# biodatageeks/datafusion-bio-functions

Hardware: AMD Instinct MI355X
Metric: overlap-pairs/sec + probe-rows/sec, IntervalJoinExec 100Mx1M (higher is better)
Workload: dtype int32; 1 GPU; join_100Mx1M_24contigs; probe_rows_per_gpu=100000000, build_rows_per_gpu=1000000, contigs=24, pairs_per_gpu=37210484, parallelism=partition-per-gpu x1, gather=False, build_overlap=True

## Files before the change

datafusion-bio-functions_amd/csrc/ivx_regions_probe.hip:

```cpp
#include "ivx_regions.hpp"
#include "ivx_agg.hpp"
#include "ivx_select.hpp"
#include "ivx_where.hpp"

namespace {


#ifndef IVX_RP_B
#define IVX_RP_B 8
#endif
#ifndef IVX_RP_RING
#define IVX_RP_RING 512
#endif
constexpr int RP_B = IVX_RP_B;
constexpr u32 RP_HALO = IVX_RP_HALO;
constexpr u32 RP_CCAP = 8192 + RP_HALO + 2;
constexpr u32 RP_RING = IVX_RP_RING;
constexpr u32 RP_NSLOT = 4;
constexpr u32 RP_NPG = 64;
constexpr u32 RP_STASH = 48;
constexpr u32 FD_SLOT_SHIFT = 13;
#ifndef IVX_FD_HEAD
#define IVX_FD_HEAD 3
#endif
constexpr int FD_HEAD = IVX_FD_HEAD;
static_assert(RP_ECAP <= (1u << FD_SLOT_SHIFT), "a slice slot must fit a stash entry's j field");
constexpr u32 RP_GRID = 256;
#ifndef IVX_RP_VGRID
#define IVX_RP_VGRID 512
#endif
constexpr u32 RP_VGRID = IVX_RP_VGRID;

struct Slice {
    const JoinIndexView *ix;
    const unsigned short *s_off; const u64 *s_ent; const u32 *s_row;
    u32 sh0, nlev, k, lb, slo, shi, e0, ncell0; bool inlds, upper, lev0;
    i32 origin; u32 span;
    i32 rbase;
    bool fast; u32 off, cmax, ncm1;
};

template <class F>
__device__ __forceinline__ void probe_row(const Slice &S, i32 qs, i32 qe, F &&f)
{
    const JoinIndexView &ix = *S.ix;
    const i64 hi64 = (i64)qe - (i64)S.origin;
    if (hi64 < 0) return;
    if (S.lev0) {
        const u32 ncell = S.ncell0;
        const i64 lo64 = (i64)qs - ((i64)1 << S.sh0) + 1 - (i64)S.origin;
        const i64 bl = lo64 <= 0 ? 0 : (lo64 >> S.sh0);
        if (bl < (i64)ncell) {
            const u32 blo = (u32)bl;
            const i64 bh = hi64 >> S.sh0;
            const u32 bhi = bh >= (i64)ncell ? ncell - 1u : (u32)bh;
            if (blo <= bhi) {
                if (S.inlds && blo >= S.slo && bhi < S.shi) {
                    const u32 a = S.s_off[blo - S.slo], b = S.s_off[bhi + 1 - S.slo];
                    for (u32 j = a; j < b; j++) {
                        const u64 x = S.s_ent[j];
                        if ((i32)(u32)x <= qe && (i32)(u32)(x >> 32) >= qs) f(j, true, (i32)(u32)x, (i32)(u32)(x >> 32));
                    }
                } else {
                    const u32 a = ix.binstart[S.lb + blo], b = ix.binstart[S.lb + bhi + 1];
                    for (u32 j = a; j < b; j++) {
                        const ivx_ent x = ix.ent[j];
                        if (x.s <= qe && x.e >= qs) f(x.row, false, x.s, x.e);
                    }
                }
            }
        }
    }
    if (S.upper) {
        for (u32 l = 1; l < S.nlev; l++) {
            if (ix.hdr[HDR_LEVCNT + l] == 0) continue;
            const u32 sh = S.sh0 + IVX_LSTEP * l;
            u32 blo = 0, bhi = 0;
            if (sh < 32) {
                const u32 ncell = (S.span >> sh) + 1u;
                const i64 lo64 = (i64)qs - ((i64)1 << sh) + 1 - (i64)S.origin;
                const i64 bl = lo64 <= 0 ? 0 : (lo64 >> sh);
                const i64 bh = hi64 >> sh;
                if (bl >= (i64)ncell) continue;
                blo = (u32)bl;
                bhi = bh >= (i64)ncell ? ncell - 1u : (u32)bh;
                if (blo > bhi) continue;
            }
            const u32 base = ix.lbase[(u64)l * ix.nkeys + S.k];
            const u32 a = ix.binstart[base + blo], b = ix.binstart[base + bhi + 1];
            for (u32 j = a; j < b; j++) {
                const ivx_ent x = ix.ent[j];
                if (x.s <= qe && x.e >= qs) f(x.row, false, x.s, x.e);
            }
        }
    }
}

template <class F>
__device__ __forceinline__ void probe_row_rel(const Slice &S, u32 rel, u32 len, bool ok, i32 qs, i32 qe, F &&f)
{
    if (S.fast && ok) {
        const u32 t = ((rel + 1u) >> S.sh0) + S.off;
        const u32 bl = t ? t - 1u : 0u;
        u32 bh = ((rel + len) >> S.sh0) + S.off;
        bh = bh < S.cmax ? bh : S.cmax;
        if (bh < S.ncm1) {
            if (bl <= bh) {
                const u32 a = S.s_off[bl], b = S.s_off[bh + 1u];
                for (u32 j = a; j < b; j++) {
                    const u64 x = S.s_ent[j];
                    if ((i32)(u32)x <= qe && (i32)(u32)(x >> 32) >= qs) f(j, true, (i32)(u32)x, (i32)(u32)(x >> 32));
                }
            }
            return;
        }
    }
    probe_row(S, qs, qe, f);
}


struct ProbeLds {
    unsigned short *s_off; u64 *s_ent; u32 *s_row;
    u64 (*s_q)[RP_RING];
    u32 *s_wpos;
    u32 (*s_wcnt)[RP_W];
    unsigned long long *s_base;
    u32 *s_arrive, *s_ready;
};

__device__ __forceinline__ void slice_init(const JoinIndexView &ix, Slice &S, const ProbeLds &L)
{
    S.ix = &ix; S.s_off = L.s_off; S.s_ent = L.s_ent; S.s_row = L.s_row;
    S.sh0 = ix.hdr[HDR_SH0]; S.nlev = ix.hdr[HDR_NLEV];
    S.upper = false;
    for (u32 l = 1; l < S.nlev; l++) S.upper |= ix.hdr[HDR_LEVCNT + l] != 0;
    S.lev0 = ix.hdr[HDR_LEVCNT] != 0;
}

__device__ __forceinline__ void slice_load(const JoinIndexView &ix, Slice &S, const ProbeLds &L, u32 r, bool reload)
{
    const u32 tid = threadIdx.x;
    __syncthreads();
    const ivx_regdesc d = ix.rdesc[r];
    S.k = d.k; S.origin = d.origin; S.span = d.span; S.lb = d.lb;
    S.ncell0 = (S.span >> S.sh0) + 1u;
    S.slo = d.slo; S.shi = d.shi; S.e0 = d.e0; S.rbase = d.rbase;
    const u32 ne = d.ne;
    const u32 nc = S.shi - S.slo + 1u;
    S.inlds = ne <= RP_ECAP && nc <= RP_CCAP;
    S.fast = S.inlds && S.lev0 && !S.upper;
    S.off = (u32)(((i64)S.rbase - (i64)S.origin) >> S.sh0) - S.slo;
    S.cmax = S.ncell0 - 1u - S.slo; S.ncm1 = S.shi - S.slo;
    if (S.inlds && reload) {
        for (u32 c0 = 0; c0 < nc; c0 += RP_T * 4) {
            u32 v[4];
#pragma unroll
            for (int u = 0; u < 4; u++) { const u32 c = c0 + u * RP_T + tid; v[u] = c < nc ? ix.binstart[S.lb + S.slo + c] : 0u; }
#pragma unroll
            for (int u = 0; u < 4; u++) { const u32 c = c0 + u * RP_T + tid; if (c < nc) L.s_off[c] = (unsigned short)(v[u] - S.e0); }
        }
        for (u32 j0 = 0; j0 < ne; j0 += RP_T * 4) {
            ivx_ent x[4];
#pragma unroll
            for (int u = 0; u < 4; u++) { const u32 j = j0 + u * RP_T + tid; if (j < ne) x[u] = ix.ent[S.e0 + j]; }
#pragma unroll
            for (int u = 0; u < 4; u++) {
                const u32 j = j0 + u * RP_T + tid;
                if (j < ne) { L.s_ent[j] = (u64)(u32)x[u].s | ((u64)(u32)x[u].e << 32); L.s_row[j] = x[u].row; }
            }
        }
    }
    __syncthreads();
}

template <bool FILL, int B, bool PK = false>
__device__ __forceinline__ u32 batch_walk(const Slice &S, const ProbeLds &L, const i32 (&qs)[B], const i32 (&qe)[B],
                                          const u32 (&rowv)[B], u32 okmask, u32 wv, u32 ring_tail, u32 &ring_start, bool &direct,
                                          const u32 (&rel)[B], const u32 (&len)[B], u32 relmask)
{
    auto walk = [&](int q, auto &&f) {
        if (PK) probe_row_rel(S, rel[q], len[q], (relmask >> q) & 1u, qs[q], qe[q], f);
        else probe_row(S, qs[q], qe[q], f);
    };
    if (!FILL) {
        u32 tsum = 0;
#pragma unroll
        for (int q = 0; q < B; q++) {
            if (!((okmask >> q) & 1u)) continue;
            walk(q, [&](u32, bool, i32, i32) { tsum++; });
        }
        return tsum;
    }
    u32 *cp = &L.s_wpos[wv];
    const u32 base = __hip_atomic_load(cp, __ATOMIC_RELAXED, __HIP_MEMORY_SCOPE_WORKGROUP);
    ring_start = base;
#pragma unroll
    for (int q = 0; q < B; q++) {
        if (!((okmask >> q) & 1u)) continue;
        walk(q, [&](u32 v, bool sl, i32, i32) {
            const u32 pos = __hip_atomic_fetch_add(cp, 1u, __ATOMIC_RELAXED, __HIP_MEMORY_SCOPE_WORKGROUP);
            if (pos - ring_tail < RP_RING)
                L.s_q[wv][pos & (RP_RING - 1)] = (u64)(sl ? S.s_row[v] : v) | ((u64)rowv[q] << 32);
        });
    }
    const u32 wtot = __hip_atomic_load(cp, __ATOMIC_RELAXED, __HIP_MEMORY_SCOPE_WORKGROUP) - base;
    direct = base + wtot - ring_tail > RP_RING;
    if (direct) ring_start = base + wtot;
    return wtot;
}

template <int B>
__device__ __forceinline__ void batch_write_direct(const Slice &S, const ProbeLds &L, const i32 (&qs)[B], const i32 (&qe)[B],
                                                   const u32 (&rowv)[B], u32 okmask, u32 wv, u64 g, bool ok, u32 *ob, u32 *op)
{
    u32 *cp = &L.s_wpos[wv];
    const u32 base = __hip_atomic_load(cp, __ATOMIC_RELAXED, __HIP_MEMORY_SCOPE_WORKGROUP);
#pragma unroll
    for (int q = 0; q < B; q++) {
        if (!((okmask >> q) & 1u)) continue;
        probe_row(S, qs[q], qe[q], [&](u32 v, bool sl, i32, i32) {
            const u32 pos = __hip_atomic_fetch_add(cp, 1u, __ATOMIC_RELAXED, __HIP_MEMORY_SCOPE_WORKGROUP) - base;
            if (ok) { ob[g + pos] = sl ? S.s_row[v] : v; op[g + pos] = rowv[q]; }
// ... 304 lines not shown
        if (t <= nreg) s_cf[t] = ex;
        __syncthreads();
        return share();
    }
    __device__ __forceinline__ bool share()
    {
        const u32 nchunk = s_cfirst[nreg];
        c_lo = (u32)((u64)nchunk * blockIdx.x / gridDim.x);
        const u32 c_hi = (u32)((u64)nchunk * (blockIdx.x + 1) / gridDim.x);
        nbatch = (c_hi - c_lo) * SUB;
        return c_lo < c_hi;
    }
    template <class Miss>
    __device__ __forceinline__ void start(Miss &&miss)
    {
        {
            u32 a = 0, b = nreg;
            while (a < b) { const u32 m = (a + b + 1) >> 1; if (s_cfirst[m] <= c_lo) a = m; else b = m - 1; }
            r = a;
        }
        src = pool;
        prefetch(0, miss);
    }
    template <class Miss>
    __device__ __forceinline__ void prefetch(u32 i, Miss &&miss)
    {
        const u32 c = c_lo + i / SUB, sb = i % SUB;
        while (c >= s_cfirst[r + 1]) r++;
        first = (c - s_cfirst[r]) * FP_CHUNK + wv * (8u * IVX_WAVE) + sb * WB;
        const u32 rows = rcur[r];
        cnt = rows > first ? (rows - first < WB ? rows - first : WB) : 0u;
        if (cnt) {
            src = routed_word(pt, pool, r, first, miss);
#pragma unroll
            for (int q = 0; q < B; q++) nx[q] = src[q * IVX_WAVE + ln];
        }
    }
    template <class Miss>
    __device__ __forceinline__ Batch take(u32 i, u32 (&rel)[B], u32 (&len)[B], u32 (&hi)[B], Miss &&miss)
    {
        const Batch b{first, cnt, src};
#pragma unroll
        for (int q = 0; q < B; q++) { const PkRow w = pk_unpack(nx[q], rowbits); rel[q] = w.rel; len[q] = w.len; hi[q] = w.hi; }
        if (i + 1 < nbatch) prefetch(i + 1, miss);
        return b;
    }
};

template <int B, bool FULL>
__device__ __forceinline__ void lean_cells_of(const Slice &S, const u32 (&rel)[B], const u32 (&len)[B], u32 maxlen, u32 cnt, u32 ln,
                                              u32 (&ca)[B], u32 (&cb)[B], u32 &slow, u32 &okm)
{
    const u32 sh0 = S.sh0, off = S.off, cmax = S.cmax, ncm1 = S.ncm1;
#pragma unroll
    for (int q = 0; q < B; q++) {
        const u32 t = ((rel[q] + 1u) >> sh0) + off;
        const u32 bl0 = (t > 1u ? t : 1u) - 1u;
        const u32 bh0 = ((rel[q] + len[q]) >> sh0) + off;
        const u32 bh = bh0 < cmax ? bh0 : cmax;
        bool bad = len[q] == maxlen || bh >= ncm1;
        const bool ok = FULL || (u32)q * IVX_WAVE + ln < cnt;
        if (ok && bad) slow |= 1u << q;
        if (ok && !bad) okm |= 1u << q;
        bad |= !ok;
        const u32 e1 = bad ? 0u : bh + 1u;
        const u32 bl = bl0 < e1 ? bl0 : e1;
        ca[q] = S.s_off[bl];
        cb[q] = S.s_off[e1];
    }
}
template <int B>
__device__ __forceinline__ void lean_cells(const Slice &S, const u32 (&rel)[B], const u32 (&len)[B], u32 maxlen, u32 cnt, u32 ln,
                                           u32 (&ca)[B], u32 (&cb)[B], u32 &slow, u32 &okm)
{
    slow = 0; okm = 0;
    if (cnt == IVX_WAVE * B) lean_cells_of<B, true>(S, rel, len, maxlen, cnt, ln, ca, cb, slow, okm);
    else lean_cells_of<B, false>(S, rel, len, maxlen, cnt, ln, ca, cb, slow, okm);
}

template <int B>
__device__ __forceinline__ void lean_list_slow(u32 slow, u32 r, u32 first, u32 ln, u64 *__restrict__ rest_rows, u32 *rest_n)
{
#pragma unroll
    for (int q = 0; q < B; q++)
        if ((slow >> q) & 1u) rest_rows[atomicAdd(rest_n + 1, 1u)] = (u64)(first + (u32)q * IVX_WAVE + ln) | ((u64)r << 32);
}

template <class W> struct RestRow { W *slot; u32 row, hi; i32 qs, qe; };
template <class W, class Miss>
__device__ __forceinline__ RestRow<W> rest_row(const JoinIndexView &ix, const PageTab &pt, W *pool, u32 r, u32 v, u32 rowbits,
                                               const i32 *ps_in, const i32 *pe_in, u32 adj, Miss &&miss)
{
    W *slot = routed_word(pt, pool, r, v, miss);
    const PkRow w = pk_unpack(*slot, rowbits);
    const u32 row = w.hi & (rowbits >= 32 ? 0xFFFFFFFFu : (1u << rowbits) - 1u);
    i32 qs, qe;
    if (w.len == pk_maxlen(rowbits)) { qs = (i32)((u32)ps_in[row] + adj); qe = (i32)((u32)pe_in[row] - adj); }
    else { qs = (i32)((u32)ix.rdesc[r].rbase + w.rel); qe = (i32)((u32)qs + w.len); }
    return RestRow<W>{slot, row, w.hi, qs, qe};
}

template <int B, bool DRAIN>
__global__ __launch_bounds__(RP_T) void k_fill_fast(JoinIndexView ix, const u64 *__restrict__ pool, const u32 *__restrict__ rcur,
                                                    PageTab pt, u32 *__restrict__ ob, u32 *__restrict__ op, u64 cap,
                                                    unsigned long long *cursor, const u32 *bsel, u32 rowbits, FpRest *__restrict__ rest, u64 *__restrict__ rest_rows, u32 *rest_n,
                                                    u32 drain)
{
    if (bsel != nullptr && *bsel != (u32)B) return;
    if (ix.hdr[HDR_SLOW] != 0u) return;
    IVX_PROBE_LDS(true)
    __shared__ u32 s_cfirst[IVX_MAXREG_WIDE + 2];
    __shared__ u32 s_wat[RP_NSLOT][RP_W];
    __shared__ u32 s_stash[DRAIN ? RP_W : 1][RP_STASH];
    const u32 wv = __builtin_amdgcn_readfirstlane(threadIdx.x / IVX_WAVE), ln = lane_id();
    auto miss = [&]() { if (ln == 0) atomicOr((unsigned int *)(cursor + 1), 1u); };
    LeanRows<B, const u64> rows;
    if (!rows.init_scan(ix, s_cfirst, &s_wat[0][0], rcur, pt, pool, rowbits)) return;
    Slice S;
    slice_init(ix, S, L);
    rows.start(miss);
    const u32 rowmask = rowbits >= 32 ? 0xFFFFFFFFu : (1u << rowbits) - 1u;
    u32 loaded_r = 0xFFFFFFFFu;
    u32 round = 0;
    u32 pend_mine = 0;
    constexpr u32 HALF = RP_RING / 2;
    auto copy_out = [&](u32 pr) {
        const u32 sl = pr % RP_NSLOT;
        while (__hip_atomic_load(&L.s_ready[sl], __ATOMIC_ACQUIRE, __HIP_MEMORY_SCOPE_WORKGROUP) != pr + 1u) __builtin_amdgcn_s_sleep(1);
        if (!pend_mine) return;
        const u64 base = L.s_base[sl];
        const u32 tot = s_wat[sl][RP_W - 1] + L.s_wcnt[sl][RP_W - 1];
        if (base + tot > cap) return;
        const u64 g = base + s_wat[sl][wv];
        u32 *ob_w = ob + g, *op_w = op + g;
        const uint2 *half = (const uint2 *)L.s_q[wv] + (pr & 1u) * HALF;
        for (u32 t = ln; t < pend_mine; t += IVX_WAVE) {
            const uint2 x = half[t];
            ob_w[t] = L.s_row[x.x]; op_w[t] = x.y & rowmask;
        }
    };
    for (u32 i = 0; i < rows.nbatch; i++) {
        const u32 r = rows.r;
        if (r != loaded_r) {
            if (round) { copy_out(round - 1u); pend_mine = 0; }
            slice_load(ix, S, L, r, true);
            loaded_r = r;
        }
        u32 rel[B], len[B], roww[B];
        const auto bt = rows.take(i, rel, len, roww, miss);
        const u32 first = bt.first, cnt = bt.cnt;
        const i32 rbase = S.rbase;
        u32 ca[B], cb[B], slow, okm;
        lean_cells<B>(S, rel, len, rows.maxlen, cnt, ln, ca, cb, slow, okm);
        u32 wpos = 0;
        uint2 *half = (uint2 *)L.s_q[wv] + (round & 1u) * HALF;
        auto step = [&](u32 &j, u32 jend, i32 qs, i32 qe, u32 rw, u64 &actm) {
            const u64 x = L.s_ent[j];
            const u64 mm = actm & __builtin_amdgcn_sicmp((i32)(u32)x, qe, 41 ) & __builtin_amdgcn_sicmp((i32)(u32)(x >> 32), qs, 39 );
            if (__builtin_amdgcn_inverse_ballot_w64(mm)) half[mask_rank_from(mm, wpos) & (HALF - 1)] = make_uint2(j, rw);
            wpos += (u32)__popcll(mm);
            j++;
            actm = __builtin_amdgcn_uicmp(j, jend, 36 );
        };
        u32 sfill = 0;
#pragma unroll
        for (int q = 0; q < B; q++) {
            const i32 qs = (i32)((u32)rbase + rel[q]), qe = (i32)((u32)qs + len[q]);
            u32 j = ca[q];
            const u32 jend = cb[q];
            u64 actm = __builtin_amdgcn_uicmp(j, jend, 36);
            if constexpr (!DRAIN) {
                if (actm != 0) {
                    do step(j, jend, qs, qe, roww[q], actm); while (actm != 0);
                }
            } else {
                const u32 lim = drain < RP_STASH - sfill ? drain : RP_STASH - sfill;
                if ((u32)__popcll(actm) > lim) {
#pragma unroll
                    for (int h = 0; h < FD_HEAD; h++) step(j, jend, qs, qe, roww[q], actm);
                    while ((u32)__popcll(actm) > lim) step(j, jend, qs, qe, roww[q], actm);
                }
                if (actm != 0) {
                    if (__builtin_amdgcn_inverse_ballot_w64(actm)) s_stash[wv][mask_rank_from(actm, sfill)] = j | (((u32)q * IVX_WAVE + ln) << FD_SLOT_SHIFT);
                    sfill += (u32)__popcll(actm);
                }
            }
        }
        if (DRAIN && sfill != 0) {
            __builtin_amdgcn_fence(__ATOMIC_RELEASE, "wavefront");
            __builtin_amdgcn_wave_barrier();
            __builtin_amdgcn_fence(__ATOMIC_ACQUIRE, "wavefront");
            const bool has = ln < sfill;
            const u32 e = has ? s_stash[wv][ln] : 0u;
            const PkRow w = pk_unpack(bt.src[e >> FD_SLOT_SHIFT], rowbits);
            const i32 qs = (i32)((u32)rbase + w.rel), qe = (i32)((u32)qs + w.len);
            const u32 bh0 = ((w.rel + w.len) >> S.sh0) + S.off;
            u32 j = e & ((1u << FD_SLOT_SHIFT) - 1u);
            const u32 jend = has ? (u32)S.s_off[(bh0 < S.cmax ? bh0 : S.cmax) + 1u] : 0u;
            u64 actm = __builtin_amdgcn_uicmp(j, jend, 36);
            while (actm != 0) step(j, jend, qs, qe, w.hi, actm);
        }
        u32 got = wpos;
        const bool skip = got > HALF;
        if (__builtin_expect(skip, 0)) {
            if (ln < B && ln * IVX_WAVE < cnt) rest[atomicAdd(rest_n, 1u)] = FpRest{r, first + ln * IVX_WAVE, cnt - ln * IVX_WAVE < IVX_WAVE ? cnt - ln * IVX_WAVE : (u32)IVX_WAVE, 0u};
            got = 0;
        } else if (__builtin_expect(slow != 0, 0)) lean_list_slow<B>(slow, r, first, ln, rest_rows, rest_n);
        if (ln == 0) {
            const u32 sl = round % RP_NSLOT;
            L.s_wcnt[sl][wv] = got;
            const u32 before = __hip_atomic_fetch_add(&L.s_arrive[sl], 1u, __ATOMIC_ACQ_REL, __HIP_MEMORY_SCOPE_WORKGROUP);
            if (before == RP_W - 1) {
                u32 tot = 0;
#pragma unroll
                for (int w = 0; w < RP_W; w++) { s_wat[sl][w] = tot; tot += L.s_wcnt[sl][w]; }
                L.s_base[sl] = tot ? atomicAdd(cursor, (unsigned long long)tot) : 0ull;
                __hip_atomic_store(&L.s_arrive[sl], 0u, __ATOMIC_RELAXED, __HIP_MEMORY_SCOPE_WORKGROUP);
                __hip_atomic_store(&L.s_ready[sl], round + 1u, __ATOMIC_RELEASE, __HIP_MEMORY_SCOPE_WORKGROUP);
            }
        }
        if (round) copy_out(round - 1u);
        pend_mine = got; round++;
    }
    if (round) copy_out(round - 1u);
}

__global__ __launch_bounds__(256) void k_fill_rest(JoinIndexView ix, const u64 *__restrict__ pool, PageTab pt, const FpRest *__restrict__ rest,
                                                   const u64 *__restrict__ rest_rows, const u32 *__restrict__ rest_n, u32 *__restrict__ ob,
                                                   u32 *__restrict__ op, u64 cap, unsigned long long *cursor, const i32 *__restrict__ ps_in,
                                                   const i32 *__restrict__ pe_in, u32 rowbits, u32 *done, u64 *host_totals)
{
    const u32 nbat = rest_n[0], nrow = rest_n[1];
    const u32 wpb = blockDim.x / IVX_WAVE, ln = lane_id();
    const u32 sh0 = ix.hdr[HDR_SH0], nlev = ix.hdr[HDR_NLEV];
    auto rows64 = [&](bool ok, u32 r, u32 v) {
        i32 qs = 0, qe = -1; u32 row = 0, k = 0;
        if (ok) {
            const auto e = rest_row(ix, pt, pool, r, v, rowbits, ps_in, pe_in, 0u, [&]() {
                const u32 was = atomicOr((unsigned int *)(cursor + 1), 1u);
                asm volatile("" ::"v"(was));
            });
            qs = e.qs; qe = e.qe; row = e.row;
            k = ix.rkey[r];
        }
        u32 m = 0;
        if (ok) walk(ix, sh0, 0, nlev, k, qs, qe, [&](u32) { m++; });
        const u32 inc = wave_incl_scan(m);
        const u32 tot = __shfl(inc, IVX_WAVE - 1, IVX_WAVE);
        if (tot == 0) return;
        unsigned long long g = 0;
        if (ln == 0) g = atomicAdd(cursor, (unsigned long long)tot);
        g = __shfl(g, 0, IVX_WAVE);
        if (g + tot > cap) return;
        u64 at = g + inc - m;
        if (m) walk(ix, sh0, 0, nlev, k, qs, qe, [&](u32 brow) { ob[at] = brow; op[at] = row; at++; });
    };
    const u32 wave = blockIdx.x * wpb + threadIdx.x / IVX_WAVE, nwave = gridDim.x * wpb;
    for (u32 i0 = wave * IVX_WAVE; i0 < nrow; i0 += nwave * IVX_WAVE) {
        const bool ok = i0 + ln < nrow;
        const u64 e = ok ? rest_rows[i0 + ln] : 0ull;
        rows64(ok, (u32)(e >> 32), (u32)e);
    }
    for (u32 b = wave; b < nbat; b += nwave) {
        const FpRest w = rest[b];
        for (u32 t0 = 0; t0 < w.cnt; t0 += IVX_WAVE) rows64(t0 + ln < w.cnt, w.r, w.first + t0 + ln);
    }
    if (host_totals == nullptr) return;
    __syncthreads();
    if (threadIdx.x == 0 && __hip_atomic_fetch_add(done, 1u, __ATOMIC_RELAXED, __HIP_MEMORY_SCOPE_AGENT) == gridDim.x - 1u) {
        host_store(host_totals, (u64)__hip_atomic_load(cursor, __ATOMIC_RELAXED, __HIP_MEMORY_SCOPE_AGENT));
        host_store(host_totals + 1, (u64)__hip_atomic_load(cursor + 1, __ATOMIC_RELAXED, __HIP_MEMORY_SCOPE_AGENT));
    }
}

#ifndef IVX_RV_WPS
#define IVX_RV_WPS 4
#endif
#ifndef IVX_RV_B
#define IVX_RV_B 8
#endif
#ifndef IVX_AGG_B
#define IVX_AGG_B 4
#endif
template <int B, class Op>
__global__ __launch_bounds__(RP_T, IVX_RV_WPS) void k_lean(JoinIndexView ix, typename Op::W *__restrict__ pool, const u32 *__restrict__ rcur, const u32 *__restrict__ cfirst,
                                               PageTab pt, u32 rowbits, u64 *__restrict__ rest_rows, u32 *rest_n, Op op)
{
    __shared__ unsigned short s_off[RP_CCAP];
    __shared__ u64 s_ent[RP_ECAP];
    __shared__ u32 s_cfirst[IVX_MAXREG_WIDE + 2];
    __shared__ typename Op::Lds s_own;
    ProbeLds L{s_off, s_ent, nullptr, nullptr, nullptr, nullptr, nullptr, nullptr, nullptr};
    const u32 ln = lane_id();
    op.begin(s_own);
    auto miss = []() {};
    LeanRows<B, typename Op::W> rows;
    if (!rows.init(ix, s_cfirst, cfirst, rcur, pt, pool, rowbits)) return;
    Slice S;
    slice_init(ix, S, L);
    rows.start(miss);
    u32 loaded_r = 0xFFFFFFFFu;
    for (u32 i = 0; i < rows.nbatch; i++) {
        const u32 r = rows.r;
        if (r != loaded_r) {
            if (loaded_r != 0xFFFFFFFFu) op.leave(ix, S, s_own);
            slice_load(ix, S, L, r, true);
            op.enter(ix, S, r, s_own);
            loaded_r = r;
        }
        u32 rel[B], len[B], roww[B];
        const auto bt = rows.take(i, rel, len, roww, miss);
        const u64 at = (u64)(bt.src - pool) + ln;
        const i32 rbase = S.rbase;
        u32 ca[B], cb[B], slow, okm;
        lean_cells<B>(S, rel, len, rows.maxlen, bt.cnt, ln, ca, cb, slow, okm);
#pragma unroll
        for (int q = 0; q < B; q++) {
            const i32 qs = (i32)((u32)rbase + rel[q]), qe = (i32)((u32)qs + len[q]);
            typename Op::Row a;
            for (u32 j = ca[q]; j < cb[q]; j++) {
                const u64 x = s_ent[j];
                const i32 xs = (i32)(u32)x, xe = (i32)(u32)(x >> 32);
                if (xs <= qe && xe >= qs) a.hit(op, s_own, j, qs, qe, xs, xe);
            }
            if ((okm >> q) & 1u) a.done(op, bt.src + q * IVX_WAVE + ln, at + (u32)q * IVX_WAVE, roww[q]);
        }
        if (__builtin_expect(slow != 0, 0)) lean_list_slow<B>(slow, r, bt.first, ln, rest_rows, rest_n);
    }
    op.leave(ix, S, s_own);
}

template <class Op>
__global__ __launch_bounds__(256) void k_lean_rest(JoinIndexView ix, typename Op::W *__restrict__ pool, PageTab pt, const u64 *__restrict__ rest_rows,
                                                   const u32 *__restrict__ rest_n, const i32 *__restrict__ ps_in, const i32 *__restrict__ pe_in,
                                                   u32 rowbits, Op op)
{
    const u32 nrow = rest_n[1];
    const u32 sh0 = ix.hdr[HDR_SH0], nlev = ix.hdr[HDR_NLEV];
    for (u32 i = blockIdx.x * blockDim.x + threadIdx.x; i < nrow; i += gridDim.x * blockDim.x) {
        const u64 ent = rest_rows[i];
        const u32 r = (u32)(ent >> 32);
        const auto e = rest_row(ix, pt, pool, r, (u32)ent, rowbits, ps_in, pe_in, op.adj, []() {});
        const i32 qs = e.qs, qe = e.qe;
        typename Op::Row a;
        if (!Op::skip_empty || !(qe < qs)) walk_ent(ix, sh0, 0, nlev, ix.rkey[r], qs, qe, [&](const ivx_ent &x) { a.hit(op, x, qs, qe); });
        a.done(op, e.slot, (u64)(e.slot - pool), e.hi);
    }
}

template <int PASS, bool IDENT, bool PAGED = false, bool PK = false>
__global__ __launch_bounds__(RP_T) void k_probe_dense(JoinIndexView ix, const void *__restrict__ rows_a, const void *__restrict__ rows_b,
                                                      const u32 *__restrict__ offs, u32 nblk, u32 prow_stride, const u32 *unsorted,
                                                      u64 *__restrict__ pcount, u32 *__restrict__ ob, u32 *__restrict__ op, u64 cap,
                                                      PageTab pt = PageTab{nullptr, 0u, 0u}, const i32 *__restrict__ ps_in = nullptr, const i32 *__restrict__ pe_in = nullptr,
                                                      u32 rowbits = 32)
{
    const u32 rowmask = rowbits >= 32 ? 0xFFFFFFFFu : (1u << rowbits) - 1u;
    const u32 maxlen = pk_maxlen(rowbits);
    if ((unsorted != nullptr && *unsorted == 0) != IDENT) return;
// ... 69 lines not shown
            }
            { const u64 g2 = g + RP_W; const u64 i2 = g2 * 64 + ln; const bool ok2 = g2 < g1 && i2 >= lo && i2 < c_hi; const u64 at = ok2 ? row_at(i2, r, rf) : 0; nx = ok2 ? row_se(at) : 0; nxr = (PASS == 1 && !PK && ok2) ? row_id(i2, at) : 0u; }
            const u64 slot = g + r;
            if (PASS == 0) {
                u32 c = 0;
                if (ok) probe_row(S, qs, qe, [&](u32, bool, i32, i32) { c++; });
                const u64 tot = wave_sum((u64)c);
                if (ln == 0) pcount[slot] = tot;
                continue;
            }
            const u64 base = __builtin_amdgcn_readfirstlane((u32)pcount[slot]) | ((u64)__builtin_amdgcn_readfirstlane((u32)(pcount[slot] >> 32)) << 32);
            u32 *const obp = ob + base, *const opp = op + base;
            const u64 room = cap > base ? cap - base : 0;
            const u32 lim = room > 0xFFFFFFFFull ? 0xFFFFFFFFu : (u32)room;
            u32 cnt = 0;
            auto walk = [&](u32 ja, u32 jb, bool lds) {
                constexpr int U = 4;
                while (__any(ja < jb)) {
                    i32 cs_[U], ce_[U]; u32 cr_[U]; bool v[U];
#pragma unroll
                    for (int u = 0; u < U; u++) {
                        v[u] = ja + u < jb;
                        cs_[u] = 0; ce_[u] = 0; cr_[u] = 0;
                        if (v[u]) {
                            if (lds) { const u64 x = S.s_ent[ja + u]; cs_[u] = (i32)(u32)x; ce_[u] = (i32)(u32)(x >> 32); cr_[u] = S.s_row[ja + u]; }
                            else { const ivx_ent x = ix.ent[ja + u]; cs_[u] = x.s; ce_[u] = x.e; cr_[u] = x.row; }
                        }
                    }
#pragma unroll
                    for (int u = 0; u < U; u++) {
                        const bool hit = v[u] && cs_[u] <= qe && ce_[u] >= qs;
                        const u64 m = __ballot(hit);
                        const u32 pos = cnt + mask_rank(m);
                        if (hit && pos < lim) { obp[pos] = cr_[u]; opp[pos] = rowv; }
                        cnt += (u32)__popcll(m);
                    }
                    ja = jb - ja > U ? ja + U : jb;
                }
            };
            const i64 hi64 = (i64)qe - (i64)S.origin;
            const bool live = ok && hi64 >= 0;
            {
                u32 ja = 0, jb = 0; bool lds = false;
                if (live && S.lev0) {
                    const u32 ncell = S.ncell0;
                    const i64 lo64 = (i64)qs - ((i64)1 << S.sh0) + 1 - (i64)S.origin;
                    const i64 bl = lo64 <= 0 ? 0 : (lo64 >> S.sh0);
                    if (bl < (i64)ncell) {
                        const u32 blo = (u32)bl;
                        const i64 bh = hi64 >> S.sh0;
                        const u32 bhi = bh >= (i64)ncell ? ncell - 1u : (u32)bh;
                        if (blo <= bhi) {
                            lds = S.inlds && blo >= S.slo && bhi < S.shi;
                            if (lds) { ja = S.s_off[blo - S.slo]; jb = S.s_off[bhi + 1 - S.slo]; }
                            else { ja = ix.binstart[S.lb + blo]; jb = ix.binstart[S.lb + bhi + 1]; }
                        }
                    }
                }
                const u32 la = lds ? ja : 0u, lb = lds ? jb : 0u, ga = lds ? 0u : ja, gb = lds ? 0u : jb;
                walk(la, lb, true);
                if (__any(ga < gb)) walk(ga, gb, false);
            }
            if (S.upper) {
                for (u32 l = 1; l < S.nlev; l++) {
                    if (ix.hdr[HDR_LEVCNT + l] == 0) continue;
                    const u32 sh = S.sh0 + IVX_LSTEP * l;
                    u32 ja = 0, jb = 0;
                    if (live) {
                        u32 blo = 0, bhi = 0; bool any = true;
                        if (sh < 32) {
                            const u32 ncell = (S.span >> sh) + 1u;
                            const i64 lo64 = (i64)qs - ((i64)1 << sh) + 1 - (i64)S.origin;
                            const i64 bl = lo64 <= 0 ? 0 : (lo64 >> sh);
                            const i64 bh = hi64 >> sh;
                            if (bl >= (i64)ncell) any = false;
                            else { blo = (u32)bl; bhi = bh >= (i64)ncell ? ncell - 1u : (u32)bh; if (blo > bhi) any = false; }
                        }
                        if (any) { const u32 lbase = ix.lbase[(u64)l * ix.nkeys + S.k]; ja = ix.binstart[lbase + blo]; jb = ix.binstart[lbase + bhi + 1]; }
                    }
                    if (__any(ja < jb)) walk(ja, jb, false);
                }
            }
        }
        lo = c_hi;
        if (PAGED && lo < hi && lo < rend) r--;
    }
}

struct RegionKnobs {
    bool two_pass;
    bool pack_off;
    bool lean_off;
    bool filter_off;
    const char *dense;
    const char *rp_rows;
    const char *fill_drain;
};
RegionKnobs region_knobs()
{
    auto is = [](const char *name, const char *v) { const char *x = getenv(name); return x && !strcmp(x, v); };
    return RegionKnobs{is("IVX_PART", "two"), is("IVX_PACK", "0"), is("IVX_FILL", "old"), is("IVX_FILTER", "0"), getenv("IVX_DENSE"), getenv("IVX_RP_ROWS"), getenv("IVX_FILL_DRAIN")};
}

int fill_rows_per_lane(const RegionKnobs &K, u64 cap, u64 n)
{
    if (K.rp_rows) return atoi(K.rp_rows);
    const double per_row = (double)cap / (double)n;
    return per_row <= 0.40 ? 8 : per_row <= 0.8 ? 4 : per_row <= 1.6 ? 2 : 1;
}

u32 fill_drain_of(const RegionKnobs &K, int b)
{
    if (K.fill_drain) { const int t = atoi(K.fill_drain); return t <= 0 ? 0u : (u32)t < RP_STASH ? (u32)t : RP_STASH; }
    return b == 8 ? 12u : b == 4 ? 16u : 0u;
}

bool dense_fill_wanted(const RegionKnobs &K, u64 cap, u64 n)
{
    if (K.dense) return atoi(K.dense) != 0;
    return (double)cap / (double)n > 3.5;
}

bool lean_rows_ok(const ivx_routed &R)
{
    return R.form == IVX_ROWS_PAGED && R.packed && R.pt.lgpg >= 13 && R.rest_rows != nullptr;
}

bool lean_fill_ok(const ivx_routed &R, const RegionKnobs &K) { return lean_rows_ok(R) && !K.lean_off && R.rest != nullptr; }

ivx_status lean_route(ivx_ctx *ctx, const JoinIndexView &jv, u32 nreg, const u32 *key, const i32 *s, const i32 *e, u64 n,
                      bool has_filter, bool pk24, bool fast, bool no_vtab, ivx_routed *R, bool *ok)
{
    *ok = false;
    const RegionKnobs K = region_knobs();
    if (n == 0 || nreg == 0 || nreg > IVX_MAXREG || !pk24 || !fast || K.two_pass || K.pack_off || K.lean_off) return IVX_OK;
    IVX_TRY(ivx_route_paged(ctx, jv, nreg, key, s, e, n, ivx_paged_opts{has_filter && !K.filter_off, true, true, true, 0u, nullptr, false, no_vtab}, R));
    *ok = lean_rows_ok(*R);
    return IVX_OK;
}

template <int B, class Op>
void lean_launch(hipStream_t st, const JoinIndexView &jv, const ivx_routed &R, const i32 *s, const i32 *e, const Op &op)
{
    typename Op::W *pool = const_cast<u64 *>(R.se);
    hipLaunchKernelGGL((k_lean<B, Op>), dim3(RP_GRID * (IVX_RV_WPS / 4)), dim3(RP_T), 0, st, jv, pool, (const u32 *)R.ctl->rcur, (const u32 *)R.ctl->cfirst, R.pt, R.rowbits,
                       R.rest_rows, R.ctl->rest_n, op);
    hipLaunchKernelGGL((k_lean_rest<Op>), dim3(256), dim3(256), 0, st, jv, pool, R.pt, (const u64 *)R.rest_rows, (const u32 *)R.ctl->rest_n, s, e, R.rowbits, op);
}

struct RecCarve {
    u8 *buf = nullptr; u64 cells = 0;
    ivx_status reserve(ivx_ctx *ctx, const ivx_routed &R, u32 nreg, u64 n, size_t cell_bytes)
    {
        cells = ((n >> R.pt.lgpg) + nreg + 1) << R.pt.lgpg;
        return ctx->get_scratch(WS_T4, (size_t)cells * cell_bytes, (void **)&buf);
    }
    template <class T> void take(T *&p, const void *wanted)
    {
        if (!wanted) return;
        p = reinterpret_cast<T *>(buf);
        buf += cells * sizeof(T);
    }
};

template <int V> using int_tag = std::integral_constant<int, V>;
template <class F> void with_rows_per_lane(int b, F &&f)
{
    switch (b) { case 1: f(int_tag<1>{}); break; case 2: f(int_tag<2>{}); break; case 4: f(int_tag<4>{}); break; default: f(int_tag<8>{}); }
}

template <int MODE, int B>
void launch_probe_regions(hipStream_t st, const JoinIndexView &jv, const ivx_routed &R, u32 grid, u32 *ob, u32 *op, u64 cap,
                          unsigned long long *cur, const u32 *bsel = nullptr, const u32 *only_if_set = nullptr)
{
    const u32 vpb = RP_VGRID / grid;
    if (R.form == IVX_ROWS_PAGED) {
        auto go = [&](auto pk) {
            hipLaunchKernelGGL((k_probe_regions<MODE, B, false, true, IVX_B(pk)>), dim3(grid), dim3(RP_T), 0, st, jv, (const void *)R.se, (const void *)R.ids, R.rfirst, 1u, vpb,
                               ob, op, cap, cur, 1u, R.adj, (const u32 *)nullptr, R.pt, bsel, R.ds, R.de, R.rowbits, only_if_set);
        };
        if constexpr (MODE >= RV_COUNT) go(std::true_type{}); else with_bools(go, R.packed);
        return;
    }
    hipLaunchKernelGGL((k_probe_regions<MODE, B, false>), dim3(grid), dim3(RP_T), 0, st, jv, (const void *)R.se, (const void *)R.ids, R.rfirst, R.nblk, vpb, ob, op, cap, cur, 1u, R.adj, R.unsorted);
    hipLaunchKernelGGL((k_probe_regions<MODE, B, true>), dim3(grid), dim3(RP_T), 0, st, jv, (const void *)R.ds, (const void *)R.de, R.rfirst, R.nblk, vpb, ob, op, cap, cur, 1u, R.adj, R.unsorted);
}

ivx_status dense_fill(ivx_ctx *ctx, const JoinIndexView &jv, u32 nreg, const ivx_routed &R, u64 n, u32 *ob, u32 *op, u64 cap, u64 *d_cursor)
{
    hipStream_t st = ctx->stream;
    const u64 slots = (n >> 6) + nreg + 3;
    u64 *pcount;
    IVX_TRY(ctx->get_scratch(WS_T3, slots * sizeof(u64), (void **)&pcount));
    IVX_HIP(ctx, hipMemsetAsync(pcount, 0, slots * sizeof(u64), st));
    auto pass = [&](auto pass_tag) {
        constexpr int P = decltype(pass_tag)::value;
        if (R.form == IVX_ROWS_PAGED) {
            with_bools([&](auto pk) {
                hipLaunchKernelGGL((k_probe_dense<P, false, true, IVX_B(pk)>), dim3(RP_VGRID), dim3(RP_T), 0, st, jv, (const void *)R.se, (const void *)R.ids, R.rfirst, 1u, 1u,
                                   (const u32 *)nullptr, pcount, ob, op, cap, R.pt, R.ds, R.de, R.rowbits);
            }, R.packed);
            return;
        }
        hipLaunchKernelGGL((k_probe_dense<P, false>), dim3(RP_VGRID), dim3(RP_T), 0, st, jv, (const void *)R.se, (const void *)R.ids, R.rfirst, R.nblk, 1u, R.unsorted, pcount, ob, op, cap);
        hipLaunchKernelGGL((k_probe_dense<P, true>), dim3(RP_VGRID), dim3(RP_T), 0, st, jv, (const void *)R.ds, (const void *)R.de, R.rfirst, R.nblk, 1u, R.unsorted, pcount, ob, op, cap);
    };
    pass(int_tag<0>{});
    IVX_TRY(ivx_scan_exclusive_u64(ctx, pcount, slots));
    IVX_HIP(ctx, hipMemcpyAsync(d_cursor, pcount + (slots - 1), sizeof(u64), hipMemcpyDeviceToDevice, st));
    pass(int_tag<1>{});
    IVX_HIP(ctx, hipGetLastError());
    return IVX_OK;
}

ivx_status probe_pairs(ivx_ctx *ctx, const JoinIndexView &jv, u32 nreg, int mode, const ivx_routed &R, u64 n, u32 *ob, u32 *op, u64 cap,
                       u64 *d_cursor, u64 hint, int fast, bool reused, const RegionKnobs &K, ivx_probe_note *note)
{
    hipStream_t st = ctx->stream;
    unsigned long long *cur = (unsigned long long *)d_cursor;
    bool due = R.tables_due;
    auto tables = [&]() -> ivx_status { if (due) { due = false; return ivx_route_paged_bounds(ctx, R, nreg); } return IVX_OK; };
    if (mode != JP_FILL) {
        IVX_TRY(tables());
        launch_probe_regions<0, RP_B>(st, jv, R, RP_VGRID, ob, op, cap, cur);
        IVX_HIP(ctx, hipGetLastError());
        return IVX_OK;
    }
    if (dense_fill_wanted(K, hint, n)) { IVX_TRY(tables()); return dense_fill(ctx, jv, nreg, R, n, ob, op, cap, d_cursor); }
    const bool paged = R.form == IVX_ROWS_PAGED;
    u32 *bsel = paged && !R.all_routed ? ctx->dword<u32>(SC_BSEL) : nullptr;
    if (bsel) IVX_TRY(tables());
    if (bsel) hipLaunchKernelGGL(k_pick_rows, dim3(1), dim3(1), 0, st, R.rfirst, nreg, hint, K.rp_rows ? (u32)atoi(K.rp_rows) : 0u, bsel);
    auto every_b = [&](auto &&f) {
        if (bsel) { f(int_tag<8>{}); f(int_tag<4>{}); f(int_tag<2>{}); f(int_tag<1>{}); }
        else with_rows_per_lane(fill_rows_per_lane(K, hint, n), f);
    };
    const u32 *slow_gate = nullptr;
    if (fast != 0 && lean_fill_ok(R, K)) {
        u32 *rest_n = R.ctl->rest_n;
        static_assert(offsetof(ivx_route_ctl, fill_done) == offsetof(ivx_route_ctl, rest_n) + 2 * sizeof(u32), "one memset clears the rest counts and the done-counter");
        if (reused) IVX_HIP(ctx, hipMemsetAsync(rest_n, 0, 3 * sizeof(u32), st));
        const bool publish = fast == 1 && note != nullptr && ctx->hd_scalars != nullptr;
        every_b([&](auto b) {
            const u32 drain = fill_drain_of(K, decltype(b)::value);
            with_bools([&](auto dr) {
                hipLaunchKernelGGL((k_fill_fast<decltype(b)::value, IVX_B(dr)>), dim3(RP_GRID), dim3(RP_T), 0, st, jv, R.se, (const u32 *)R.ctl->rcur, R.pt, ob, op, cap, cur,
                                   (const u32 *)bsel, R.rowbits, R.rest, R.rest_rows, rest_n, drain);
            }, drain != 0);
        });
        hipLaunchKernelGGL(k_fill_rest, dim3(512), dim3(256), 0, st, jv, R.se, R.pt, (const FpRest *)R.rest, (const u64 *)R.rest_rows, (const u32 *)rest_n, ob, op, cap, cur, R.ds, R.de, R.rowbits,
                           &R.ctl->fill_done, publish ? ctx->hdword(SC_PAIRS) : (u64 *)nullptr);
        IVX_HIP(ctx, hipGetLastError());
        if (publish) note->totals_on_host = true;
        if (fast == 1) return IVX_OK;
        slow_gate = jv.hdr + HDR_SLOW;
    }
    IVX_TRY(tables());
    every_b([&](auto b) { launch_probe_regions<1, decltype(b)::value>(st, jv, R, RP_GRID, ob, op, cap, cur, bsel, slow_gate); });
    IVX_HIP(ctx, hipGetLastError());
    return IVX_OK;
}

}

ivx_status ivx_join_probe_regions(ivx_ctx *ctx, const JoinIndexView &jv, u32 nreg, int mode,
                                  const u32 *key, const i32 *s, const i32 *e, u64 n,
                                  u32 *ob, u32 *op, u64 cap, u64 *d_cursor, bool planned, bool has_filter, bool pk24, int fast, hipEvent_t ready, bool clear_cursor,
                                  ivx_probe_note *note)
{
    auto wait_ready = [&]() -> ivx_status { if (ready) { IVX_HIP(ctx, hipStreamWaitEvent(ctx->stream, ready, 0)); ready = nullptr; } return IVX_OK; };
    const RegionKnobs K = region_knobs();
    const bool paged_route = !planned && n != 0 && nreg <= IVX_MAXREG_WIDE && !K.two_pass;
    if (clear_cursor && !paged_route) IVX_HIP(ctx, hipMemsetAsync(d_cursor, 0, 2 * sizeof(u64), ctx->stream));
    if (n == 0) return wait_ready();
    ivx_join_plan &pl = ctx->join_plan;
    ivx_routed R;
    if (planned) R = pl.rows;
    else {
        if (nreg > IVX_MAXREG_WIDE) {
            IVX_TRY(wait_ready());
            IVX_TRY(ivx_route_two_level(ctx, jv, nreg, key, s, e, n, &R));
        } else if (K.two_pass) {
            IVX_TRY(wait_ready());
            IVX_TRY(ivx_route_flat(ctx, jv, key, s, e, n, 0u, nreg > IVX_MAXREG ? 1024u : 256u, false, 4, &R));
        } else {
            const bool bounds_due = mode == JP_FILL && !(has_filter && !K.filter_off);
            IVX_TRY(ivx_route_paged(ctx, jv, nreg, key, s, e, n, ivx_paged_opts{has_filter && !K.filter_off, pk24 && !K.pack_off, false, fast != 0, 0u, clear_cursor ? d_cursor : nullptr, bounds_due}, &R));
            if (fast == 2 && ready != nullptr && note != nullptr && note->ix_serial != 0 && ctx->hdr_mirror_serial == note->ix_serial) {
                IVX_HIP(ctx, hipEventSynchronize(ready));
                fast = ctx->hword<u32>(SC_HDR_MIRROR)[HDR_SLOW] == 0 ? 1 : 0;
                note->fast = fast;
            }
        }
        if (mode == JP_COUNT) { pl.rows = R; pl.valid = true; }
    }
    IVX_TRY(wait_ready());
    const u64 hint = ctx->fill_hint ? ctx->fill_hint : (planned && pl.total < cap ? pl.total : cap);
    return probe_pairs(ctx, jv, nreg, mode, R, n, ob, op, cap, d_cursor, hint, fast, planned, K, note);
}

// ... 88 lines not shown
```

Baseline: 38.61 billion overlap-pairs/s.

## Prune look-back cell scan using per-cell reach class packed into staged offsets

When a bin slice is staged in LDS, each cell's offset entry now carries a 3-bit class in its high bits giving how far that cell's intervals reach into the next cell, in eighths of a cell. The lean cell-range computation uses this class to skip the preceding cell when the probe start lies beyond that reach, cutting candidate entries that cannot overlap. It also adds a separate head-step count for B=8 in the fill stash drain. The cost is an extra pass over entries at slice load plus masking on every offset read; an env knob disables the pruning.

```diff
diff --git a/datafusion-bio-functions_amd/csrc/ivx_regions_probe.hip b/datafusion-bio-functions_amd/csrc/ivx_regions_probe.hip
--- a/datafusion-bio-functions_amd/csrc/ivx_regions_probe.hip
+++ b/datafusion-bio-functions_amd/csrc/ivx_regions_probe.hip
@@ -24,7 +24,14 @@
 #define IVX_FD_HEAD 3
 #endif
 constexpr int FD_HEAD = IVX_FD_HEAD;
-static_assert(RP_ECAP <= (1u << FD_SLOT_SHIFT), "a slice slot must fit a stash entry's j field");
+#ifndef IVX_FD_HEAD8
+#define IVX_FD_HEAD8 2
+#endif
+constexpr int FD_HEAD8 = IVX_FD_HEAD8;
+constexpr u32 RP_OFF_MASK = 0x1FFFu;
+constexpr u32 RP_CLS_SHIFT = 13;
+static_assert(RP_ECAP <= (1u << FD_SLOT_SHIFT) && RP_ECAP <= RP_OFF_MASK && RP_OFF_MASK == (1u << RP_CLS_SHIFT) - 1u,
+              "a slice slot must fit a stash entry's j field and a staged cell offset's low bits");
 constexpr u32 RP_GRID = 256;
 #ifndef IVX_RP_VGRID
 #define IVX_RP_VGRID 512
@@ -39,6 +46,8 @@
     i32 rbase;
     bool fast; u32 off, cmax, ncm1;
 };
+
+__device__ __forceinline__ u32 slice_off(const unsigned short *s_off, u32 c) { return (u32)s_off[c] & RP_OFF_MASK; }
 
 template <class F>
 __device__ __forceinline__ void probe_row(const Slice &S, i32 qs, i32 qe, F &&f)
@@ -56,7 +65,7 @@
             const u32 bhi = bh >= (i64)ncell ? ncell - 1u : (u32)bh;
             if (blo <= bhi) {
                 if (S.inlds && blo >= S.slo && bhi < S.shi) {
-                    const u32 a = S.s_off[blo - S.slo], b = S.s_off[bhi + 1 - S.slo];
+                    const u32 a = slice_off(S.s_off, blo - S.slo), b = slice_off(S.s_off, bhi + 1 - S.slo);
                     for (u32 j = a; j < b; j++) {
                         const u64 x = S.s_ent[j];
                         if ((i32)(u32)x <= qe && (i32)(u32)(x >> 32) >= qs) f(j, true, (i32)(u32)x, (i32)(u32)(x >> 32));
@@ -106,7 +115,7 @@
         bh = bh < S.cmax ? bh : S.cmax;
         if (bh < S.ncm1) {
             if (bl <= bh) {
-                const u32 a = S.s_off[bl], b = S.s_off[bh + 1u];
+                const u32 a = slice_off(S.s_off, bl), b = slice_off(S.s_off, bh + 1u);
                 for (u32 j = a; j < b; j++) {
                     const u64 x = S.s_ent[j];
                     if ((i32)(u32)x <= qe && (i32)(u32)(x >> 32) >= qs) f(j, true, (i32)(u32)x, (i32)(u32)(x >> 32));
@@ -137,7 +146,8 @@
     S.lev0 = ix.hdr[HDR_LEVCNT] != 0;
 }
 
-__device__ __forceinline__ void slice_load(const JoinIndexView &ix, Slice &S, const ProbeLds &L, u32 r, bool reload)
+enum : u32 { CLS_NONE = 0, CLS_SEVEN = 1, CLS_REACH = 2 };
+__device__ __forceinline__ void slice_load(const JoinIndexView &ix, Slice &S, const ProbeLds &L, u32 r, bool reload, u32 cls = CLS_NONE)
 {
     const u32 tid = threadIdx.x;
     __syncthreads();
@@ -168,6 +178,26 @@
                 const u32 j = j0 + u * RP_T + tid;
                 if (j < ne) { L.s_ent[j] = (u64)(u32)x[u].s | ((u64)(u32)x[u].e << 32); L.s_row[j] = x[u].row; }
             }
+        }
+        if (cls != CLS_NONE) {
+            __syncthreads();
+            const bool exact = cls == CLS_REACH && S.sh0 >= 3u && S.sh0 < 32u;
+            const u32 sh3 = exact ? S.sh0 - 3u : 0u, full = exact ? (1u << S.sh0) - 1u : 0u;
+            const u32 *ends = (const u32 *)L.s_ent + 1;
+            for (u32 c = tid; c + 1u < nc; c += RP_T) {
+                const u32 a = slice_off(L.s_off, c), b = slice_off(L.s_off, c + 1u);
+                u32 q = 7u;
+                if (exact) {
+                    const u32 first = (S.slo + c) << S.sh0;
+                    u32 far = 0;
+                    for (u32 j = a; j < b; j++) { const u32 d = ends[2u * j] - (u32)S.origin - first; far = d > far ? d : far; }
+                    const u32 reach = far > full ? far - full : 0u;
+                    const u32 k = ((reach - 1u) >> sh3) + 1u;
+                    q = reach == 0u ? 0u : k < 7u ? k : 7u;
+                }
+                L.s_off[c] = (unsigned short)(a | (q << RP_CLS_SHIFT));
+            }
+            if (tid == 0 && nc < RP_CCAP) L.s_off[nc] = (unsigned short)ne;
         }
     }
     __syncthreads();
@@ -578,21 +608,36 @@
                                               u32 (&ca)[B], u32 (&cb)[B], u32 &slow, u32 &okm)
 {
     const u32 sh0 = S.sh0, off = S.off, cmax = S.cmax, ncm1 = S.ncm1;
-#pragma unroll
-    for (int q = 0; q < B; q++) {
-        const u32 t = ((rel[q] + 1u) >> sh0) + off;
-        const u32 bl0 = (t > 1u ? t : 1u) - 1u;
-        const u32 bh0 = ((rel[q] + len[q]) >> sh0) + off;
-        const u32 bh = bh0 < cmax ? bh0 : cmax;
-        bool bad = len[q] == maxlen || bh >= ncm1;
-        const bool ok = FULL || (u32)q * IVX_WAVE + ln < cnt;
-        if (ok && bad) slow |= 1u << q;
-        if (ok && !bad) okm |= 1u << q;
-        bad |= !ok;
-        const u32 e1 = bad ? 0u : bh + 1u;
-        const u32 bl = bl0 < e1 ? bl0 : e1;
-        ca[q] = S.s_off[bl];
-        cb[q] = S.s_off[e1];
+    const u32 sh3 = sh0 >= 3u ? sh0 - 3u : 0u;
+    constexpr int G = B < 4 ? B : 4;
+#pragma unroll
+    for (int g = 0; g < B; g += G) {
+        u32 nx[G], back = 0;
+#pragma unroll
+        for (int q = g; q < g + G; q++) {
+            const u32 own = (rel[q] >> sh0) + off;
+            const u32 bl0 = (own > 1u ? own : 1u) - 1u;
+            const u32 bh0 = ((rel[q] + len[q]) >> sh0) + off;
+            const u32 bh = bh0 < cmax ? bh0 : cmax;
+            bool bad = len[q] == maxlen || bh >= ncm1;
+            const bool ok = FULL || (u32)q * IVX_WAVE + ln < cnt;
+            if (ok && bad) slow |= 1u << q;
+            if (ok && !bad) okm |= 1u << q;
+            bad |= !ok;
+            const u32 e1 = bad ? 0u : bh + 1u;
+            const u32 bl = bl0 < e1 ? bl0 : e1;
+            if (bl < own) back |= 1u << (q - g);
+            ca[q] = S.s_off[bl];
+            nx[q - g] = S.s_off[bl + 1u];
+            cb[q] = S.s_off[e1];
+        }
+#pragma unroll
+        for (int q = g; q < g + G; q++) {
+            const u32 u8th = (rel[q] >> sh3) & 7u;
+            const bool skip = (((back >> (q - g)) & 1u) != 0u) & ((u8th < 6u ? u8th : 6u) >= (ca[q] >> RP_CLS_SHIFT));
+            ca[q] = (skip ? nx[q - g] : ca[q]) & RP_OFF_MASK;
+            cb[q] &= RP_OFF_MASK;
+        }
     }
 }
 template <int B>
@@ -630,7 +675,7 @@
 __global__ __launch_bounds__(RP_T) void k_fill_fast(JoinIndexView ix, const u64 *__restrict__ pool, const u32 *__restrict__ rcur,
                                                     PageTab pt, u32 *__restrict__ ob, u32 *__restrict__ op, u64 cap,
                                                     unsigned long long *cursor, const u32 *bsel, u32 rowbits, FpRest *__restrict__ rest, u64 *__restrict__ rest_rows, u32 *rest_n,
-                                                    u32 drain)
+                                                    u32 drain, u32 prune)
 {
     if (bsel != nullptr && *bsel != (u32)B) return;
     if (ix.hdr[HDR_SLOW] != 0u) return;
@@ -669,7 +714,7 @@
         const u32 r = rows.r;
         if (r != loaded_r) {
             if (round) { copy_out(round - 1u); pend_mine = 0; }
-            slice_load(ix, S, L, r, true);
+            slice_load(ix, S, L, r, true, prune != 0u ? CLS_REACH : CLS_SEVEN);
             loaded_r = r;
         }
         u32 rel[B], len[B], roww[B];
@@ -703,7 +748,7 @@
                 const u32 lim = drain < RP_STASH - sfill ? drain : RP_STASH - sfill;
                 if ((u32)__popcll(actm) > lim) {
 #pragma unroll
-                    for (int h = 0; h < FD_HEAD; h++) step(j, jend, qs, qe, roww[q], actm);
+                    for (int h = 0; h < (B == 8 ? FD_HEAD8 : FD_HEAD); h++) step(j, jend, qs, qe, roww[q], actm);
                     while ((u32)__popcll(actm) > lim) step(j, jend, qs, qe, roww[q], actm);
                 }
                 if (actm != 0) {
@@ -722,7 +767,7 @@
             const i32 qs = (i32)((u32)rbase + w.rel), qe = (i32)((u32)qs + w.len);
             const u32 bh0 = ((w.rel + w.len) >> S.sh0) + S.off;
             u32 j = e & ((1u << FD_SLOT_SHIFT) - 1u);
-            const u32 jend = has ? (u32)S.s_off[(bh0 < S.cmax ? bh0 : S.cmax) + 1u] : 0u;
+            const u32 jend = has ? slice_off(S.s_off, (bh0 < S.cmax ? bh0 : S.cmax) + 1u) : 0u;
             u64 actm = __builtin_amdgcn_uicmp(j, jend, 36);
             while (actm != 0) step(j, jend, qs, qe, w.hi, actm);
         }
@@ -810,7 +855,7 @@
 #endif
 template <int B, class Op>
 __global__ __launch_bounds__(RP_T, IVX_RV_WPS) void k_lean(JoinIndexView ix, typename Op::W *__restrict__ pool, const u32 *__restrict__ rcur, const u32 *__restrict__ cfirst,
-                                               PageTab pt, u32 rowbits, u64 *__restrict__ rest_rows, u32 *rest_n, Op op)
+                                               PageTab pt, u32 rowbits, u64 *__restrict__ rest_rows, u32 *rest_n, u32 prune, Op op)
 {
     __shared__ unsigned short s_off[RP_CCAP];
     __shared__ u64 s_ent[RP_ECAP];
@@ -830,7 +875,7 @@
         const u32 r = rows.r;
         if (r != loaded_r) {
             if (loaded_r != 0xFFFFFFFFu) op.leave(ix, S, s_own);
-            slice_load(ix, S, L, r, true);
+            slice_load(ix, S, L, r, true, prune != 0u ? CLS_REACH : CLS_SEVEN);
             op.enter(ix, S, r, s_own);
             loaded_r = r;
         }
@@ -1006,7 +1051,7 @@
                         const u32 bhi = bh >= (i64)ncell ? ncell - 1u : (u32)bh;
                         if (blo <= bhi) {
                             lds = S.inlds && blo >= S.slo && bhi < S.shi;
-                            if (lds) { ja = S.s_off[blo - S.slo]; jb = S.s_off[bhi + 1 - S.slo]; }
+                            if (lds) { ja = slice_off(S.s_off, blo - S.slo); jb = slice_off(S.s_off, bhi + 1 - S.slo); }
                             else { ja = ix.binstart[S.lb + blo]; jb = ix.binstart[S.lb + bhi + 1]; }
                         }
                     }
@@ -1049,11 +1094,13 @@
     const char *dense;
     const char *rp_rows;
     const char *fill_drain;
+    bool prune_off;
 };
 RegionKnobs region_knobs()
 {
     auto is = [](const char *name, const char *v) { const char *x = getenv(name); return x && !strcmp(x, v); };
-    return RegionKnobs{is("IVX_PART", "two"), is("IVX_PACK", "0"), is("IVX_FILL", "old"), is("IVX_FILTER", "0"), getenv("IVX_DENSE"), getenv("IVX_RP_ROWS"), getenv("IVX_FILL_DRAIN")};
+    return RegionKnobs{is("IVX_PART", "two"), is("IVX_PACK", "0"), is("IVX_FILL", "old"), is("IVX_FILTER", "0"), getenv("IVX_DENSE"), getenv("IVX_RP_ROWS"), getenv("IVX_FILL_DRAIN"),
+                       is("IVX_LOOKBACK_PRUNE", "0")};
 }
 
 int fill_rows_per_lane(const RegionKnobs &K, u64 cap, u64 n)
@@ -1097,8 +1144,9 @@
 void lean_launch(hipStream_t st, const JoinIndexView &jv, const ivx_routed &R, const i32 *s, const i32 *e, const Op &op)
 {
     typename Op::W *pool = const_cast<u64 *>(R.se);
+    const u32 prune = region_knobs().prune_off ? 0u : 1u;
     hipLaunchKernelGGL((k_lean<B, Op>), dim3(RP_GRID * (IVX_RV_WPS / 4)), dim3(RP_T), 0, st, jv, pool, (const u32 *)R.ctl->rcur, (const u32 *)R.ctl->cfirst, R.pt, R.rowbits,
-                       R.rest_rows, R.ctl->rest_n, op);
+                       R.rest_rows, R.ctl->rest_n, prune, op);
     hipLaunchKernelGGL((k_lean_rest<Op>), dim3(256), dim3(256), 0, st, jv, pool, R.pt, (const u64 *)R.rest_rows, (const u32 *)R.ctl->rest_n, s, e, R.rowbits, op);
 }
 
@@ -1199,7 +1247,7 @@
             const u32 drain = fill_drain_of(K, decltype(b)::value);
             with_bools([&](auto dr) {
                 hipLaunchKernelGGL((k_fill_fast<decltype(b)::value, IVX_B(dr)>), dim3(RP_GRID), dim3(RP_T), 0, st, jv, R.se, (const u32 *)R.ctl->rcur, R.pt, ob, op, cap, cur,
-                                   (const u32 *)bsel, R.rowbits, R.rest, R.rest_rows, rest_n, drain);
+                                   (const u32 *)bsel, R.rowbits, R.rest, R.rest_rows, rest_n, drain, K.prune_off ? 0u : 1u);
             }, drain != 0);
         });
         hipLaunchKernelGGL(k_fill_rest, dim3(512), dim3(256), 0, st, jv, R.se, R.pt, (const FpRest *)R.rest, (const u64 *)R.rest_rows, (const u32 *)rest_n, ob, op, cap, cur, R.ds, R.de, R.rowbits,
```

Measured after the change: 38.85 billion overlap-pairs/s, median of 6. About the same (+0.6%).
